# Kmatsuo57/cell-image-analysis

Hardware: AMD Instinct MI355X
Metric: cells/sec screened (CAE fwd + recon-MSE + SVM score), 64x64 (higher is better)
Workload: dtype f32 (results in the fp32 error class; the contractions run as split 16-bit products on the matrix pipe, fp32 accumulate: conv1..conv6 as 2 fp16 terms x 3 products with exact power-of-two scales from each cell's own data, the PCA GEMM as 3 bf16 terms x 6 products, conv7's 32 -> 16 channel contraction; 1 GPU; BASELINE.json configs[2]: screening inference, 1000000 synthetic 64x64 crops on one GPU, resident in HBM, CAE fwd + recon MSE/MAE + RobustScaler + PCA(100) + 2x OCSVM score on device; cells_per_gpu=1000000, global_cells=1000000, chunk_cells=65536, detector_train_cells=5000, weights=random init (Glorot, non-trivial BN), seed 42, parallelism=dp1

## Files before the change

cell-image-analysis_amd/cellscreen/_lib.py:

```python
from __future__ import annotations

import ctypes as C
import os
from typing import Optional

import numpy as np

CS_MAX_CONV = 16
CS_MEM_HOST, CS_MEM_DEVICE = 0, 1
_PKG = os.path.dirname(os.path.dirname(os.path.abspath(__file__)))
LIB_PATH = os.path.join(_PKG, "libcellscreen.so")


class CellScreenError(RuntimeError):
    def __init__(self, status: int, message: str):
        super().__init__(f"libcellscreen status {status}: {message}")
        self.status = status


class CSAugAffine(C.Structure):
    _fields_ = [("m", C.c_double * 4), ("off", C.c_double * 2), ("identity", C.c_int32), ("flip_h", C.c_int32),
                ("flip_v", C.c_int32), ("reserved", C.c_int32)]


# ... 178 lines not shown
                                   C.POINTER(CSBackgroundParams), _P, _I]),
    "cs_segment_background_last_timing": (_I, [_P, C.POINTER(C.c_double), C.POINTER(C.c_double)]),
    "cs_segment_local": (_I, [_P, _P, _I, C.c_int32, C.c_int32, C.c_int32, C.c_int32, C.c_int32, _I, C.POINTER(CSLocalParams), _P, _I]),
    "cs_segment_local_last_timing": (_I, [_P, C.POINTER(C.c_double), C.POINTER(C.c_double)]),
    "cs_segment_clean": (_I, [_P, _P, _I, C.c_int32, C.c_int32, C.c_int32, C.c_int32, C.c_int32, _I, C.POINTER(CSSegmentParams),
                              C.POINTER(CSCleanParams), _P, _I, _P]),
    "cs_segment_clean_last_timing": (_I, [_P, C.POINTER(C.c_double), C.POINTER(C.c_double), C.POINTER(C.c_double)]),
    "cs_segment_hysteresis": (_I, [_P, _P, _I, C.c_int32, C.c_int32, C.c_int32, C.c_int32, C.c_int32, _I, C.POINTER(CSSegmentParams),
                                   C.POINTER(CSLocalParams), C.POINTER(CSHysteresisParams), _P, _I, _P]),
    "cs_segment_hysteresis_last_timing": (_I, [_P, C.POINTER(C.c_double), C.POINTER(C.c_double)]),
    "cs_segment_noise": (_I, [_P, _P, _I, C.c_int32, C.c_int32, C.c_int32, C.c_int32, C.c_int32, _I, C.POINTER(CSNoiseParams), _P, _I, _P]),
    "cs_segment_noise_last_timing": (_I, [_P, C.POINTER(C.c_double), C.POINTER(C.c_double), C.POINTER(C.c_double)]),
    "cs_segment_smooth": (_I, [_P, _P, _I, C.c_int32, C.c_int32, C.c_int32, C.c_int32, C.c_int32, _I, C.POINTER(CSSmoothParams), _P, _I]),
    "cs_segment_smooth_last_timing": (_I, [_P, C.POINTER(C.c_double), C.POINTER(C.c_double)]),
    "cs_label_match": (_I, [_P, _P, _P, C.c_int32, C.c_int32, C.c_int32, _I, C.c_int32, C.c_int32, C.POINTER(CSMatchParams), _P, _P, _I, _P]),
    "cs_label_match_last_timing": (_I, [_P, C.POINTER(C.c_double), C.POINTER(C.c_double)]),
    "cs_label_match_last_table": (_I, [_P, C.POINTER(C.c_int32), C.POINTER(C.c_int32)]),
    "cs_label_expand": (_I, [_P, _P, C.c_int32, C.c_int32, C.c_int32, _I, C.POINTER(CSExpandParams), _P, _P, _I]),
    "cs_label_expand_last_timing": (_I, [_P, C.POINTER(C.c_double), C.POINTER(C.c_double)]),
    "cs_label_intensity": (_I, [_P, _P, _I, C.c_int32, _P, _P, C.c_int32, C.c_int32, C.c_int32, _I, C.c_int32, _P, _P, _I]),
    "cs_label_intensity_last_timing": (_I, [_P, C.POINTER(C.c_double), C.POINTER(C.c_double)]),
    "cs_label_quantiles": (_I, [_P, _P, _I, C.c_int32, _P, _P, C.c_int32, C.c_int32, C.c_int32, _I, C.c_int32, _P, _P, C.c_int32, _I,
                                _P, _P, _P, _I]),
    "cs_label_quantiles_last_timing": (_I, [_P, C.POINTER(C.c_double), C.POINTER(C.c_double), C.POINTER(C.c_double)]),
    "cs_label_texture": (_I, [_P, _P, _I, C.c_int32, _P, _P, C.c_int32, C.c_int32, C.c_int32, _I, C.c_int32, C.c_int32, C.c_int32, _P, _P,
                              _P, _P, _P, _P, _P, _I]),
    "cs_label_texture_last_timing": (_I, [_P, C.POINTER(C.c_double), C.POINTER(C.c_double)]),
    "cs_label_shape": (_I, [_P, _P, _P, C.c_int32, C.c_int32, C.c_int32, _I, C.c_int32, _I, _P, _P, _P, _P, _P, _I]),
    "cs_label_shape_last_timing": (_I, [_P, C.POINTER(C.c_double), C.POINTER(C.c_double)]),
    "cs_label_neighbors": (_I, [_P, _P, C.c_int32, C.c_int32, C.c_int32, _I, C.c_int32, C.POINTER(CSNeighborsParams), _P, _P, _P, _I,
                           C.POINTER(_L)]),
    "cs_label_neighbors_pairs": (_I, [_P, _P, _L, _I]),
    "cs_label_neighbors_last_timing": (_I, [_P, C.POINTER(C.c_double), C.POINTER(C.c_double)]),
    "cs_label_neighbors_last_table": (_I, [_P, C.POINTER(C.c_int32), C.POINTER(C.c_int32)]),
    "cs_fit_create": (_I, [_I, C.POINTER(_P)]),
    "cs_fit_free": (None, [_P]),
    "cs_fit_wait_stream": (_I, [_P, _P]),
    "cs_fit_scaler": (_I, [_P, _P, _L, C.c_int32, _I, _P, _P]),
    "cs_fit_pca_moments": (_I, [_P, _P, _L, C.c_int32, _I, _P, _P, _P, _P]),
    "cs_fit_pca_subspace": (_I, [_P, _P, _L, C.c_int32, _I, _P, _P, C.c_int32, C.c_uint64, _P, _P, _P, C.POINTER(C.c_double),
                                 C.POINTER(C.c_int32)]),
    "cs_fit_project": (_I, [_P, _P, _L, C.c_int32, _I, _P, _P, _P, _P, C.c_int32, _P]),
    "cs_fit_ocsvm": (_I, [_P, _P, _L, C.c_int32, C.c_double, C.c_double, C.c_double, _L, _P, C.POINTER(C.c_double),
                          C.POINTER(C.c_double), C.POINTER(_L), C.POINTER(C.c_int32)]),
    "cs_fit_last_ms": (_I, [_P, C.POINTER(C.c_double)]),
    "cs_synth_crops": (_I, [_P, C.c_uint64, _L, _L, C.c_int32, _P]),
    "cs_profile_enable": (_I, [_P, _I]),
    "cs_profile_reset": (_I, [_P]),
    "cs_profile_kernel_count": (_I, []),
    "cs_profile_kernel_name": (C.c_char_p, [_I]),
    "cs_profile_get": (_I, [_P, _I, C.POINTER(C.c_double), C.POINTER(_L), C.POINTER(_L), C.POINTER(C.c_double)]),
    "cs_profile_mfma_per_cell": (_I, [_P, _I, C.POINTER(C.c_double)]),
    "cs_profile_bf16_mfma_per_cell": (_I, [_P, _I, C.POINTER(C.c_double)]),
    "cs_train_param_count": (_I, [C.POINTER(_L), C.POINTER(_L)]),
    "cs_train_param_count_of": (_I, [_P, C.POINTER(_L), C.POINTER(_L)]),
    "cs_train_create": (_I, [C.POINTER(CSCaeWeights), C.POINTER(CSTrainCfg), _I, C.POINTER(_P)]),
    "cs_train_free": (None, [_P]),
    "cs_train_wait_stream": (_I, [_P, _P]),
    "cs_train_step": (_I, [_P, _P, _P, _L, _I, C.c_float, C.POINTER(C.c_float), C.POINTER(C.c_float)]),
    "cs_train_step_async": (_I, [_P, _P, _P, _L, _I, C.c_float]),
    "cs_train_inputs_consumed": (_I, [_P, _P]),
    "cs_train_draw_transforms": (_I, [C.POINTER(CSAugConfig), C.c_uint64, C.c_uint64, _L, C.c_int32, C.c_int32, _P]),
    "cs_train_fit_step": (_I, [_P, _P, _L, _P, _L, C.POINTER(CSAugConfig), C.c_uint64, C.c_uint64, C.c_float]),
    "cs_train_read_metrics": (_I, [_P, C.POINTER(C.c_double), C.POINTER(C.c_double), C.POINTER(_L), _I]),
    "cs_train_forward_backward": (_I, [_P, _P, _P, _L, _I, C.POINTER(C.c_float), C.POINTER(C.c_float)]),
    "cs_train_apply": (_I, [_P, C.c_float]),
    "cs_train_set_grad_buffer": (_I, [_P, _P]),
    "cs_train_set_sync_bn": (_I, [_P, _P, _P, _P, _L, _I, _I]),
    "cs_train_set_sync_bn_stream": (_I, [_P, _P, _P, _P, _L, _I, _I]),
    "cs_train_eval": (_I, [_P, _P, _P, _L, _I, C.POINTER(C.c_float), C.POINTER(C.c_float)]),
    "cs_train_augment": (_I, [_P, _P, _L, _P, _P, _I]),
    "cs_train_export": (_I, [_P, _P, _P, _P]),
    "cs_train_tensor": (_I, [_P, _I, _I, _L, _P]),
    "cs_train_import": (_I, [_P, _P, _P]),
}

_lib = None


def load_library(path: Optional[str] = None):
    global _lib
    if _lib is not None:
        return _lib
    path = path or LIB_PATH
    if not os.path.exists(path):
        raise FileNotFoundError(f"{path} not built; run `python cell-image-analysis_amd/build.py` "
                                "(or __graft_entry__.build()).  There is no CPU fallback.")
    try:
        import torch
    except Exception:
        pass
    lib = C.CDLL(path, mode=C.RTLD_GLOBAL)
    for name, (res, args) in SIGNATURES.items():
        fn = getattr(lib, name)
        fn.restype = res
        fn.argtypes = args
    if lib.cs_abi_version() != 2:
        raise RuntimeError("libcellscreen ABI version mismatch")
    _lib = lib
    return lib


def check(status: int):
    if status != 0:
        lib = load_library()
        msg = lib.cs_last_error().decode(errors="replace") or lib.cs_status_string(status).decode()
# ... 44 lines not shown
```

cell-image-analysis_amd/cellscreen/engine.py:

```python
from __future__ import annotations

import ctypes as C
from typing import Dict, Optional

import numpy as np

from . import _lib as L
from . import spec
from .spec import CAEWeights, DetectorParams


def _fill_cae(w: CAEWeights, keep: list) -> L.CSCaeWeights:
    s = L.CSCaeWeights()
    s.height, s.width = w.input_hw
    s.n_conv, s.n_enc = w.n_conv, w.n_enc
    s.bn_eps = w.bn_eps

    def put(field, l, arr):
        a = np.ascontiguousarray(arr, dtype=np.float32)
        keep.append(a)
        getattr(s, field)[l] = a.ctypes.data

    for l in range(w.n_conv):
        s.channels[l] = w.channels[l]
# ... 126 lines not shown

    def encode(self, crops, which: int = 1):
        buf, n, kind = self._crops(crops)
        f = self._alloc(kind, buf, (n, self.info.feature_dim), np.float32)
        L.check(self._lib.cs_encode(self._h, L._ptr(buf), n, kind, which, L._ptr(f), kind))
        return f

    def layer_output(self, crops, layer: int):
        buf, n, kind = self._crops(crops)
        rows = spec.layer_table((self.info.height, self.info.width), tuple(self.info.channels[:self.info.n_conv]), self.info.n_enc)
        oh, ow = rows[layer]["out_hw"]
        o = self._alloc(kind, buf, (n, oh, ow, rows[layer]["cout"]), np.float32)
        L.check(self._lib.cs_layer_output(self._h, L._ptr(buf), n, kind, layer, L._ptr(o), kind))
        return o

    def scaler_pca(self, features: np.ndarray) -> np.ndarray:
        f = np.ascontiguousarray(features, dtype=np.float32)
        o = np.empty((f.shape[0], self.info.n_components), dtype=np.float32)
        L.check(self._lib.cs_scaler_pca(self._h, f.ctypes.data, f.shape[0], L.CS_MEM_HOST, o.ctypes.data, L.CS_MEM_HOST))
        return o

    def svm_decision(self, pca: np.ndarray):
        p = np.ascontiguousarray(pca, dtype=np.float32)
        c = np.empty(p.shape[0], dtype=np.float64)
        m = np.empty(p.shape[0], dtype=np.float64)
        L.check(self._lib.cs_svm_decision(self._h, p.ctypes.data, p.shape[0], L.CS_MEM_HOST, c.ctypes.data, m.ctypes.data, L.CS_MEM_HOST))
        return c, m

    def synth_crops(self, seed: int, first_cell: int, out_tensor):
        n = out_tensor.shape[0]
        npix = int(np.prod(out_tensor.shape[1:]))
        L.order_after_torch(self._lib.cs_model_wait_stream, self._h, out_tensor)
        L.check(self._lib.cs_synth_crops(self._h, seed, first_cell, n, npix, out_tensor.data_ptr()))
        return out_tensor

    def profile_enable(self, on: bool = True):
        L.check(self._lib.cs_profile_enable(self._h, 1 if on else 0))

    def profile_reset(self):
        L.check(self._lib.cs_profile_reset(self._h))

    def profile(self) -> Dict[str, dict]:
        out = {}
        for k in range(self._lib.cs_profile_kernel_count()):
            ms, ln, cells, fl = C.c_double(), C.c_int64(), C.c_int64(), C.c_double()
            L.check(self._lib.cs_profile_get(self._h, k, C.byref(ms), C.byref(ln), C.byref(cells), C.byref(fl)))
            mf = C.c_double()
            L.check(self._lib.cs_profile_mfma_per_cell(self._h, k, C.byref(mf)))
            bf = C.c_double()
            L.check(self._lib.cs_profile_bf16_mfma_per_cell(self._h, k, C.byref(bf)))
            out[self._lib.cs_profile_kernel_name(k).decode()] = dict(ms=ms.value, launches=ln.value, cells=cells.value, flops=fl.value,
                                                                      mfma_per_cell=mf.value, bf16_mfma_per_cell=bf.value)
        return out
```

cell-image-analysis_amd/csrc/api.hip:

```cpp
#include "api_internal.hpp"
#include "tensor_archive.hpp"

using namespace cs;

static thread_local std::string g_err;

namespace cs {
int fail(int code, const char* fmt, ...)
{
    char buf[1024];
    va_list ap;
    va_start(ap, fmt);
    vsnprintf(buf, sizeof buf, fmt, ap);
    va_end(ap);
    g_err = buf;
    return code;
}
const char* last_error_cstr() { return g_err.c_str(); }
}

static const char* kKernelNames[K_COUNT] = {"conv1_relu_bn_pool", "conv2_relu_bn_pool", "conv3_relu_bn_pool",
                                            "conv4_relu_bn",      "conv5_up_relu_bn",   "conv6_up_relu_bn",
                                            "conv7_up_sigmoid_err", "scaler_pca",       "ocsvm_decision",
                                            "finalize",           "synth_crops",        "conv6_conv7_fused_err",
// ... 1143 lines not shown
    if ((rc = ensure_workspace(m, ch, false))) return rc;
    double* outs[2] = {cons_dec, mod_dec};
    for (int64_t off = 0; off < n; off += ch) {
        const int64_t nc = (n - off) < ch ? (n - off) : ch;
        const float* p;
        if ((rc = stage_in(m, pca, in_kind, off, nc, (size_t)m->C, m->pca, &p))) return rc;
        for (int d = 0; d < 2; ++d) {
            if (!outs[d]) continue;
            LAUNCH(K_SVM, nc,
                   launch_ocsvm(p, m->C, m->svm[d].svT.as<double>(), m->svm[d].svn.as<double>(), m->svm[d].coef.as<double>(),
                                m->svm[d].nsv_pad, m->svm[d].gamma, m->svm[d].rho, m->dec[d].as<double>(), nc, m->stream, m->det_ws.p));
            HIPCHK(hipMemcpyAsync(outs[d] + off, m->dec[d].p, (size_t)nc * sizeof(double),
                                  out_kind == CS_MEM_DEVICE ? hipMemcpyDeviceToDevice : hipMemcpyDeviceToHost, m->stream));
        }
        HIPCHK(hipStreamSynchronize(m->stream));
    }
    return guard.done(end_call(m));
}

int cs_synth_crops(cs_model* m, uint64_t seed, int64_t first_cell, int64_t n, int32_t npix, float* out_device)
{
    int rc = begin_call(m);
    if (rc) return rc;
    if (n < 0 || npix <= 0) return fail(CS_ERR_INVALID, "n/npix invalid");
    if (n == 0) return CS_OK;
    if (!out_device) return fail(CS_ERR_INVALID, "out_device is NULL");
    LAUNCH(K_SYNTH, n, launch_synth(seed, first_cell, n, npix, out_device, m->stream));
    return end_call(m);
}

int cs_profile_enable(cs_model* m, int on)
{
    if (!m) return fail(CS_ERR_INVALID, "model handle is NULL");
    m->prof = on != 0;
    return CS_OK;
}

int cs_profile_reset(cs_model* m)
{
    if (!m) return fail(CS_ERR_INVALID, "model handle is NULL");
    for (int k = 0; k < K_COUNT; ++k) { m->prof_ms[k] = 0; m->prof_launches[k] = 0; m->prof_cells[k] = 0; }
    return CS_OK;
}

int cs_model_wait_stream(cs_model* m, void* hip_stream)
{
    if (!m) return fail(CS_ERR_INVALID, "model handle is NULL");
    HIPCHK(hipSetDevice(m->device));
    return wait_on_stream(m->stream, hip_stream);
}

int cs_profile_kernel_count(void) { return K_COUNT; }

const char* cs_profile_kernel_name(int k) { return (k >= 0 && k < K_COUNT) ? kKernelNames[k] : ""; }

int cs_profile_get(cs_model* m, int k, double* total_ms, int64_t* launches, int64_t* cells, double* flops)
{
    if (!m || k < 0 || k >= K_COUNT) return fail(CS_ERR_INVALID, "bad kernel id");
    if (total_ms) *total_ms = m->prof_ms[k];
    if (launches) *launches = m->prof_launches[k];
    if (cells) *cells = m->prof_cells[k];
    if (flops) {
        double per_cell = 0.0;
        if (k <= K_CONV7_ERR) per_cell = 2.0 * kLayerMacs[k];
        else if (k == K_CONV67_FUSED) per_cell = 2.0 * (kLayerMacs[5] + kLayerMacs[6]);
        else if (k == K_CONV12_FUSED) per_cell = 2.0 * (kLayerMacs[0] + kLayerMacs[1]);
        else if (k == K_SCALER_PCA) per_cell = 2.0 * (double)m->F * m->C;
        else if (k == K_SVM) per_cell = 0.0;
        *flops = per_cell * (double)m->prof_cells[k];
    }
    return CS_OK;
}

int cs_profile_mfma_per_cell(cs_model* m, int k, double* mfma)
{
    if (!m || !mfma || k < 0 || k >= K_COUNT) return fail(CS_ERR_INVALID, "bad kernel id");
    double v = 0.0;
    if (k == K_SCALER_PCA) {
        *mfma = m->has_det && !m->split16 ? (double)m->fpad * m->cpad / 1024.0 : 0.0;
        return CS_OK;
    }
    if (m->arch.ref) {
        const bool h2 = m->split16;
        switch (k) {
            case K_CONV1: v = 1536; break;
            case K_CONV2: v = 8192; break;
            case K_CONV3: v = h2 ? 0 : 2048; break;
            case K_CONV4: v = h2 ? 0 : 576; break;
            case K_CONV5: v = h2 ? 0 : 1152; break;
            case K_CONV6: v = 4608; break;
            case K_CONV67_FUSED: v = h2 ? 512 : 4608 + 512; break;
            case K_CONV12_FUSED: v = h2 ? 0 : 4608 + 1536 + 48; break;
            default: v = 0.0;
        }
    } else if (k <= K_CONV6 || k == K_CONV7_ERR) {
        const int l = k == K_CONV7_ERR ? m->arch.n_conv - 1 : k - K_CONV1;
        if (l < m->arch.n_conv && !(m->split16 && m->gae.x3[l])) {
            const int cout_pad = (m->arch.ch[l] + 15) / 16 * 16;
            v = (double)m->arch.gh[l] * m->arch.gw[l] / 16.0 * (cout_pad / 16) * (9.0 * m->arch.cin(l) / 4.0);
        }
    }
    *mfma = v;
    return CS_OK;
}

int cs_profile_bf16_mfma_per_cell(cs_model* m, int k, double* mfma)
// ... 29 lines not shown
```

cell-image-analysis_amd/csrc/common.hpp:

```cpp
#pragma once
#include <hip/hip_runtime.h>
#include <stdint.h>
#include <stdio.h>

#include "../../include/cellscreen.h"

namespace cs {

typedef float f32x4 __attribute__((ext_vector_type(4)));

struct LayerGeom {
    int H, W, cin, cout;
    bool pool;
    bool ups;
    bool last;
};

enum KernelId {
    K_CONV1 = 0, K_CONV2, K_CONV3, K_CONV4, K_CONV5, K_CONV6, K_CONV7_ERR,
    K_SCALER_PCA, K_SVM, K_FINALIZE, K_SYNTH, K_CONV67_FUSED, K_CONV12_FUSED, K_COUNT
};

hipError_t launch_conv_mfma(int layer, const float* in, const float* wfrag, const float* ep,
                            float* out, int64_t n_cells, hipStream_t stream, bool folded = false);
size_t pack_conv_fragments_folded(int cin, int cout, const float* hwio, float* dst);
hipError_t launch_conv_wino_cs(int layer, const float* in, const float* ufrag, const float* ep, float* out, int64_t n_cells,
                               hipStream_t stream);
size_t pack_wino_cs_fragments(int layer, const float* hwio, float* dst);
hipError_t launch_conv3_wino_h2(const float* in, const uint16_t* uplanes, float inv_sw, const float* ep, float* out, int64_t n_cells,
                                hipStream_t stream);
size_t pack_wino3_h2(const float* hwio, uint16_t* dst, float* inv_sw);
hipError_t launch_conv12_fused(const float* x, const float* w1frag, const float* ep1, const float* ufrag, const float* ep2, float* p2,
                               int64_t n_cells, hipStream_t stream, const unsigned int* ufrag_h2 = nullptr,
                               float p1a = 0.0f, float p1b = 0.0f, float inv_sw = 1.0f, const unsigned int* w1h2 = nullptr, float inv_sw1 = 1.0f);
size_t pack_conv12_conv1_h2(const float* hwio, const float* bn_scale, unsigned int* dst, float* inv_sw1);
size_t pack_conv12_fragments_h2(const float* hwio, const float* bn_scale, unsigned int* dst, float* inv_sw);
void pack_conv12_p1_bound(const float* hwio1, const float* ep1, float* a1, float* b1);
size_t pack_conv12_fragments(const float* hwio, const float* bn_scale, float* dst);
size_t pack_conv12_conv1_fragments(const float* hwio, const float* bn_scale, float* dst);
hipError_t launch_conv4_h2(const float* in, const uint16_t* wfrag, float inv_sw, const float* ep, float* out, int64_t n_cells, hipStream_t stream);
size_t pack_conv4_f16x2(const float* hwio, uint16_t* dst, float* inv_sw);
hipError_t launch_conv5_h2(const float* in, const uint16_t* wfrag, float inv_sw, const float* ep, float* out, int64_t n_cells, hipStream_t stream);
hipError_t launch_conv45_h2(const float* in, const uint16_t* w4, float inv_sw4, const float* ep4, const uint16_t* w5, float inv_sw5,
                            const float* ep5, float* out, int64_t n_cells, hipStream_t stream);
size_t pack_conv5_f16x2(const float* weff, uint16_t* dst, float* inv_sw);
hipError_t launch_conv_wino_up(int layer, const float* in, const float* ufrag, const float* ep, float* out, int64_t n_cells,
                               hipStream_t stream);
size_t pack_wino_up_fragments(int layer, const float* hwio, float* dst);
size_t pack_conv_fragments(int cin, int cout, const float* hwio, float* dst);

hipError_t launch_conv67_fused(const float* a5, const float* ufrag, const float* ep, const float* x, const float* weff_dev,
                               const float* b7_dev, float* errpart, int64_t n_cells, hipStream_t stream);
int conv67_fused_nparts();
hipError_t launch_conv67_h2(const float* a5, const uint16_t* wplanes, float inv_sw, const float* ep, const float* x, const float* weff_dev,
                            const float* b7_dev, float* errpart, int64_t n_cells, hipStream_t stream);
size_t pack_conv6_f16x2(const float* weff, uint16_t* dst, float* inv_sw);

hipError_t launch_conv7_err(const float* a6, const float* x, const float* weff_dev, const float* b7_dev,
                            float* errpart, float* recon, int64_t n_cells, hipStream_t stream);
hipError_t launch_conv7_err_train(const float* a6, const float* x, const float* weff_dev, const float* b7_dev, float* errpart,
                                  float* recon, float* dz, float* dzsum_part, int64_t n_cells, hipStream_t stream);
void conv7_effective_weights(const float* w7_hwio, float* weff);

constexpr int TRAIN_MAX_PARTS = 256;
constexpr int BN_MAX_PARTS = 1024;
struct ReduceDesc { long dst; long len; const float* src; int nparts; long stride; };
hipError_t launch_conv_train_fwd(int layer, const float* in, const float* wfrag, const float* bias,
                                 float* relu_out, int64_t n_cells, hipStream_t stream, float* stats_part = nullptr,
                                 int* stats_parts = nullptr);
hipError_t launch_conv_dgrad(int layer, const float* dz, const float* wfrag_t, float* dx, int64_t n_cells,
                             hipStream_t stream);
hipError_t launch_bn_stats(const float* r, long P, int C, float* part, int* G, hipStream_t s);
hipError_t launch_bn_stats_final(const float* part, int G, int C, float eps, float momentum, float* mov_mean,
                                 float* mov_var, float* stats, hipStream_t s);
hipError_t launch_bn_stats_merge(const float* part, int G, int C, float* out , hipStream_t s);
hipError_t launch_bn_apply(const float* r, int C, const float* gamma, const float* beta, const float* stats, float* a,
                           long N, int H, int W, int pool, hipStream_t s);
hipError_t launch_loss_dz(const float* out, const float* y, long total, float* dz, float* dzsum_part, int* G, hipStream_t s,
                          const float* errpart = nullptr, long nparts = 0, float* out2 = nullptr);
hipError_t launch_loss_scalar(const float* errpart, long nparts, long nelem, float* out2, hipStream_t s);
hipError_t launch_bn_bwd_reduce(const float* da, const float* r, const float* stats, const float* gamma, const float* beta,
                                long N, int H, int W, int C, int pool, float* part, int* G, hipStream_t s);
hipError_t launch_bn_bwd_final(const float* part, int G, int C, double nred, float* sums, float* dgamma, float* dbeta,
                               hipStream_t s);
hipError_t launch_bn_bwd_dz(const float* da, const float* r, const float* stats, const float* gamma, const float* beta,
                            const float* sums, long N, int H, int W, int C, int pool, float* dz, float* dzsum_part,
                            int* Gz, hipStream_t s);
hipError_t launch_wgrad(int layer, const float* xin, const float* dz, float* part, int64_t n_cells, int* nparts,
                        hipStream_t s);
hipError_t launch_reduce_all(const ReduceDesc* descs_dev, int ndesc, long total_len, float* flat_grad, hipStream_t s,
                             const float* errpart = nullptr, long nparts = 0, long nelem = 0, float* out2 = nullptr);
hipError_t launch_adam(float* p, const float* g, float* m, float* v, long n, float alpha, float b1, float b2, float eps, hipStream_t s,
                       const float* batch_scal, double* macc);
enum { GEN_EPI_BN = 0, GEN_EPI_BN_POOL = 1, GEN_EPI_SIGMOID = 2, GEN_EPI_RELU = 3, GEN_EPI_PLAIN = 4 };
int conv_generic_supported(int H, int W, int cin, int cout, char* why, size_t why_len);
hipError_t launch_conv_generic(const float* in, const float* w_hwio, const float* ep, float* out, int64_t n, int H, int W, int cin,
                               int cout, int ups, int epi, hipStream_t stream, const float* w_folded = nullptr);
// ... 58 lines not shown
```

cell-image-analysis_amd/csrc/conv45_h2.hip:

```cpp
#include "kernel_setup.hpp"
#include "split16.hpp"

#include <cstring>

namespace cs {

namespace {

constexpr int G = 8;
constexpr int CH = 32;
constexpr int WP = G + 2;
constexpr int PXB = 64;
constexpr int ROWB = WP * PXB + 32;
constexpr int PLANE = WP * ROWB;
constexpr int WG_PER_CU = 2;

constexpr int C5_OUT = 64;

constexpr int H2_OFF_MAX = 2 * PLANE;
constexpr int H2_LDS_BYTES = 2 * PLANE + 16;

__device__ __forceinline__ void h2_split_store(char* dst, const f32x4& x, float S)
{
    f16x4 hi;
// ... 139 lines not shown
    __syncthreads();
    float S, invS;
    f16x2_scale(mxw[0], S, invS);
    const int woff = ((tid >> 6) + 1) * ROWB + (((tid >> 3) & 7) + 1) * PXB + (tid & 7) * 8;
    const int abase = ((li >> 3) + pa) * ROWB + ((li & 7) + pb) * PXB + kq * 16;

    for (int it = 0; cell < n_cells; cell += gridDim.x, ++it) {
        const float unscale = invS * inv_sw;
        h2_split_store(smem + woff, stg, S);
        __syncthreads();
        if (tid == 0) mxw[it & 1] = 0;
        const long ncell = cell + gridDim.x;
        if (ncell < n_cells) stg = *(const f32x4*)(in + (size_t)ncell * (G * G * CH) + tid * 4);

        float* obase = out + (((size_t)cell * (2 * G) + pa) * (2 * G) + pb) * C5_OUT + (2 * sp) * 16 + li;
#pragma unroll
        for (int t = 0; t < 4; ++t) {
            f32x4 ah[2] = {{0.0f, 0.0f, 0.0f, 0.0f}, {0.0f, 0.0f, 0.0f, 0.0f}};
            f32x4 al[2] = {{0.0f, 0.0f, 0.0f, 0.0f}, {0.0f, 0.0f, 0.0f, 0.0f}};
#pragma unroll
            for (int tap = 0; tap < 4; ++tap) {
                const char* a = smem + abase + t * (2 * ROWB) + (tap >> 1) * ROWB + (tap & 1) * PXB;
                const f16x8 a1 = *(const f16x8*)a;
                const f16x8 a2 = *(const f16x8*)(a + PLANE);
#pragma unroll
                for (int k = 0; k < 2; ++k) {
                    al[k] = __builtin_amdgcn_mfma_f32_16x16x32_f16(a1, B[tap][k][1], al[k], 0, 0, 0);
                    ah[k] = __builtin_amdgcn_mfma_f32_16x16x32_f16(a1, B[tap][k][0], ah[k], 0, 0, 0);
                    al[k] = __builtin_amdgcn_mfma_f32_16x16x32_f16(a2, B[tap][k][0], al[k], 0, 0, 0);
                }
            }
#pragma unroll
            for (int r = 0; r < 4; ++r) {
                const int i = 4 * kq + r, ys = 2 * t + (i >> 3), xs = i & 7;
                float* o = obase + ((size_t)(2 * ys) * (2 * G) + 2 * xs) * C5_OUT;
#pragma unroll
                for (int k = 0; k < 2; ++k) {
                    const float v = fmaxf(fmaf(ah[k][r] + al[k][r], unscale, bias[k]), 0.0f);
                    o[16 * k] = fmaf(v, bns[k], bnt[k]);
                }
            }
        }
        if (ncell < n_cells) {
            unsigned int mx = 0;
            f16x2_absmax4(stg, mx);
            mx = f16x2_rowmax(mx);
            if (li == 0) atomicMax(&mxw[(it + 1) & 1], mx);
        }
        __syncthreads();
        f16x2_scale(mxw[(it + 1) & 1], S, invS);
    }
}

constexpr int F45_OFF_A = 2 * PLANE;
constexpr int F45_OFF_W4 = 4 * PLANE;
constexpr int F45_W4_BYTES = 2 * 9 * 2 * 64 * 16;
constexpr int F45_OFF_MAX = F45_OFF_W4 + F45_W4_BYTES;
constexpr int F45_LDS_BYTES = F45_OFF_MAX + 16;
static_assert(2 * F45_LDS_BYTES <= 160 * 1024, "two workgroups per CU");

__global__ __launch_bounds__(512, 2) void conv45_h2_kernel(const float* __restrict__ in , const f16x8* __restrict__ w4frag,
                                                           const float* __restrict__ ep4, float inv_sw4, const f16x8* __restrict__ w5frag,
                                                           const float* __restrict__ ep5, float inv_sw5, float* __restrict__ out ,
                                                           long n_cells)
{
    extern __shared__ __attribute__((aligned(16))) char smem[];
    unsigned int* const mxw = (unsigned int*)(smem + F45_OFF_MAX);
    const int tid = threadIdx.x;
    const int lane = tid & 63;
    const int wave = __builtin_amdgcn_readfirstlane(tid >> 6);
    const int li = lane & 15, kq = lane >> 4;
    const int ph = wave >> 1, pa = ph >> 1, pb = ph & 1;
    const int sp = wave & 1;
    const int slice4 = wave & 1, tile4 = wave >> 1;

    f16x8 B[4][2][2];
#pragma unroll
    for (int t = 0; t < 4; ++t)
#pragma unroll
        for (int k = 0; k < 2; ++k)
#pragma unroll
            for (int p = 0; p < 2; ++p) B[t][k][p] = w5frag[(((wave * 4 + t) * 2 + k) * 2 + p) * 64 + lane];
    float bias[2], bns[2], bnt[2];
#pragma unroll
    for (int k = 0; k < 2; ++k) {
        const int co = (2 * sp + k) * 16 + li;
        bias[k] = ep5[co]; bns[k] = ep5[C5_OUT + co]; bnt[k] = ep5[2 * C5_OUT + co];
    }
    const int co4 = slice4 * 16 + li;
    const float bias4 = ep4[co4], bns4 = ep4[CH + co4], bnt4 = ep4[2 * CH + co4];

    for (int i = tid; i < F45_LDS_BYTES / 16; i += 512) *(f32x4*)(smem + i * 16) = f32x4{0.0f, 0.0f, 0.0f, 0.0f};
    __syncthreads();
    for (int i = tid; i < F45_W4_BYTES / 16; i += 512) *(f16x8*)(smem + F45_OFF_W4 + i * 16) = w4frag[i];

    long cell = blockIdx.x;
    if (cell >= n_cells) return;
    f32x4 stg = *(const f32x4*)(in + (size_t)cell * (G * G * CH) + tid * 4);
    {
        unsigned int mx = 0;
        f16x2_absmax4(stg, mx);
        mx = f16x2_rowmax(mx);
        if (li == 0) atomicMax(&mxw[0], mx);
    }
    __syncthreads();
    float S3, invS3;
    f16x2_scale(mxw[0], S3, invS3);
    const int woff = ((tid >> 6) + 1) * ROWB + (((tid >> 3) & 7) + 1) * PXB + (tid & 7) * 8;
    const int abase4 = (2 * tile4 + (li >> 3)) * ROWB + (li & 7) * PXB + kq * 16;
    const char* const w4l = smem + F45_OFF_W4 + (size_t)slice4 * 9 * 2 * 64 * 16 + lane * 16;
    const int abase5 = F45_OFF_A + ((li >> 3) + pa) * ROWB + ((li & 7) + pb) * PXB + kq * 16;

    for (int it = 0; cell < n_cells; cell += gridDim.x, ++it) {
        h2_split_store(smem + woff, stg, S3);
        __syncthreads();
        if (tid == 0) mxw[it & 1] = 0;
        const long ncell = cell + gridDim.x;
        if (ncell < n_cells) stg = *(const f32x4*)(in + (size_t)ncell * (G * G * CH) + tid * 4);

        f32x4 a4v;
        {
            f32x4 hi = {0.0f, 0.0f, 0.0f, 0.0f}, lo = {0.0f, 0.0f, 0.0f, 0.0f};
#pragma unroll
            for (int tap = 0; tap < 9; ++tap) {
                const char* a = smem + abase4 + (tap / 3) * ROWB + (tap % 3) * PXB;
                const f16x8 a1 = *(const f16x8*)a;
                const f16x8 a2 = *(const f16x8*)(a + PLANE);
                const f16x8 bh = *(const f16x8*)(w4l + (tap * 2 + 0) * 1024), bl = *(const f16x8*)(w4l + (tap * 2 + 1) * 1024);
                lo = __builtin_amdgcn_mfma_f32_16x16x32_f16(a1, bl, lo, 0, 0, 0);
                hi = __builtin_amdgcn_mfma_f32_16x16x32_f16(a1, bh, hi, 0, 0, 0);
                lo = __builtin_amdgcn_mfma_f32_16x16x32_f16(a2, bh, lo, 0, 0, 0);
            }
            const float us4 = invS3 * inv_sw4;
            float am = 0.0f;
#pragma unroll
            for (int r = 0; r < 4; ++r) {
                const float v = fmaxf(fmaf(hi[r] + lo[r], us4, bias4), 0.0f);
                a4v[r] = fmaf(v, bns4, bnt4);
                am = fmaxf(am, fabsf(a4v[r]));
            }
            const unsigned int m = f16x2_rowmax(__builtin_bit_cast(unsigned int, am));
            if (li == 0) atomicMax(&mxw[2 + (it & 1)], m);
        }
        __syncthreads();
        float S4, invS4;
        f16x2_scale(mxw[2 + (it & 1)], S4, invS4);
        {
#pragma unroll
            for (int r = 0; r < 4; ++r) {
                const int p = 16 * tile4 + 4 * kq + r;
                char* d = smem + F45_OFF_A + ((p >> 3) + 1) * ROWB + ((p & 7) + 1) * PXB + co4 * 2;
                const float v = a4v[r] * S4;
                const _Float16 h = (_Float16)v;
                *(_Float16*)d = h;
                *(_Float16*)(d + PLANE) = (_Float16)(v - (float)h);
            }
        }
        __syncthreads();
        if (tid == 0) mxw[2 + (it & 1)] = 0;

        const float unscale = invS4 * inv_sw5;
        float* obase = out + (((size_t)cell * (2 * G) + pa) * (2 * G) + pb) * C5_OUT + (2 * sp) * 16 + li;
#pragma unroll
        for (int t = 0; t < 4; ++t) {
            f32x4 ah[2] = {{0.0f, 0.0f, 0.0f, 0.0f}, {0.0f, 0.0f, 0.0f, 0.0f}};
            f32x4 al[2] = {{0.0f, 0.0f, 0.0f, 0.0f}, {0.0f, 0.0f, 0.0f, 0.0f}};
#pragma unroll
            for (int tap = 0; tap < 4; ++tap) {
                const char* a = smem + abase5 + t * (2 * ROWB) + (tap >> 1) * ROWB + (tap & 1) * PXB;
                const f16x8 a1 = *(const f16x8*)a;
                const f16x8 a2 = *(const f16x8*)(a + PLANE);
#pragma unroll
                for (int k = 0; k < 2; ++k) {
                    al[k] = __builtin_amdgcn_mfma_f32_16x16x32_f16(a1, B[tap][k][1], al[k], 0, 0, 0);
                    ah[k] = __builtin_amdgcn_mfma_f32_16x16x32_f16(a1, B[tap][k][0], ah[k], 0, 0, 0);
                    al[k] = __builtin_amdgcn_mfma_f32_16x16x32_f16(a2, B[tap][k][0], al[k], 0, 0, 0);
                }
            }
#pragma unroll
            for (int r = 0; r < 4; ++r) {
                const int i = 4 * kq + r, ys = 2 * t + (i >> 3), xs = i & 7;
                float* o = obase + ((size_t)(2 * ys) * (2 * G) + 2 * xs) * C5_OUT;
#pragma unroll
                for (int k = 0; k < 2; ++k) {
                    const float v = fmaxf(fmaf(ah[k][r] + al[k][r], unscale, bias[k]), 0.0f);
                    o[16 * k] = fmaf(v, bns[k], bnt[k]);
                }
            }
        }
        if (ncell < n_cells) {
            unsigned int mx = 0;
            f16x2_absmax4(stg, mx);
            mx = f16x2_rowmax(mx);
            if (li == 0) atomicMax(&mxw[(it + 1) & 1], mx);
        }
        __syncthreads();
        f16x2_scale(mxw[(it + 1) & 1], S3, invS3);
    }
}

}

size_t pack_conv4_f16x2(const float* hwio, uint16_t* dst, float* inv_sw)
{
    const size_t n = (size_t)2 * 9 * 2 * 64 * 8;
    if (!dst) return n;
    const float S = f16x2_weight_scale(hwio, (size_t)9 * CH * CH);
    if (inv_sw) *inv_sw = 1.0f / S;
    for (int s = 0; s < 2; ++s)
        for (int t = 0; t < 9; ++t)
            for (int l = 0; l < 64; ++l)
                for (int j = 0; j < 8; ++j) {
                    const int li = l & 15, kq = l >> 4;
                    uint16_t pl[2];
                    f16x2_split(hwio[((size_t)t * CH + 8 * kq + j) * CH + 16 * s + li], S, pl[0], pl[1]);
                    for (int p = 0; p < 2; ++p) dst[((((size_t)s * 9 + t) * 2 + p) * 64 + l) * 8 + j] = pl[p];
                }
    return n;
}

hipError_t launch_conv4_h2(const float* in, const uint16_t* wfrag, float inv_sw, const float* ep, float* out, int64_t n_cells, hipStream_t stream)
{
    if (n_cells <= 0) return hipSuccess;
    KernelSetup ks;
    if (hipError_t e = kernel_setup<conv4_h2_kernel>(256, H2_LDS_BYTES, ks); e != hipSuccess) return e;
    const long grid = n_cells < ks.resident ? n_cells : ks.resident;
    hipLaunchKernelGGL(conv4_h2_kernel, dim3((unsigned)grid), dim3(256), H2_LDS_BYTES, stream, in, (const f16x8*)wfrag, ep, out,
                       (long)n_cells, inv_sw);
    return hipGetLastError();
}

size_t pack_conv5_f16x2(const float* weff, uint16_t* dst, float* inv_sw)
{
    const size_t n = (size_t)8 * 4 * 2 * 2 * 64 * 8;
    if (!dst) return n;
    const float S = f16x2_weight_scale(weff, (size_t)16 * CH * C5_OUT);
    if (inv_sw) *inv_sw = 1.0f / S;
    for (int w = 0; w < 8; ++w)
        for (int t = 0; t < 4; ++t)
            for (int k = 0; k < 2; ++k)
                for (int l = 0; l < 64; ++l)
                    for (int j = 0; j < 8; ++j) {
                        const int ph = w >> 1, sp = w & 1, li = l & 15, kq = l >> 4;
                        uint16_t pl[2];
                        f16x2_split(weff[((size_t)(ph * 4 + t) * CH + 8 * kq + j) * C5_OUT + (2 * sp + k) * 16 + li], S, pl[0], pl[1]);
                        for (int p = 0; p < 2; ++p) dst[((((((size_t)w * 4 + t) * 2 + k) * 2 + p) * 64) + l) * 8 + j] = pl[p];
                    }
    return n;
}

hipError_t launch_conv5_h2(const float* in, const uint16_t* wfrag, float inv_sw, const float* ep, float* out, int64_t n_cells, hipStream_t stream)
{
    if (n_cells <= 0) return hipSuccess;
    KernelSetup ks;
    if (hipError_t e = kernel_setup<conv5_h2_kernel>(512, H2_LDS_BYTES, ks); e != hipSuccess) return e;
    const long grid = n_cells < ks.resident ? n_cells : ks.resident;
    hipLaunchKernelGGL(conv5_h2_kernel, dim3((unsigned)grid), dim3(512), H2_LDS_BYTES, stream, in, (const f16x8*)wfrag, ep, out,
                       (long)n_cells, inv_sw);
    return hipGetLastError();
}

hipError_t launch_conv45_h2(const float* in, const uint16_t* w4, float inv_sw4, const float* ep4, const uint16_t* w5, float inv_sw5,
                            const float* ep5, float* out, int64_t n_cells, hipStream_t stream)
{
    if (n_cells <= 0) return hipSuccess;
    KernelSetup ks;
    if (hipError_t e = kernel_setup<conv45_h2_kernel>(512, F45_LDS_BYTES, ks); e != hipSuccess) return e;
    const long grid = n_cells < ks.resident ? n_cells : ks.resident;
    hipLaunchKernelGGL(conv45_h2_kernel, dim3((unsigned)grid), dim3(512), F45_LDS_BYTES, stream, in, (const f16x8*)w4, ep4, inv_sw4,
                       (const f16x8*)w5, ep5, inv_sw5, out, (long)n_cells);
    return hipGetLastError();
}

}
```

include/cellscreen.h:

```cpp
#ifndef CELLSCREEN_H
#define CELLSCREEN_H

#include <stdint.h>

#ifdef __cplusplus
extern "C" {
#endif

#define CS_ABI_VERSION 2
#define CS_MAX_CONV 16

typedef enum cs_status {
    CS_OK = 0,
    CS_ERR_INVALID = -1,
    CS_ERR_IO = -2,
    CS_ERR_FORMAT = -3,
    CS_ERR_NO_DEVICE = -4,
    CS_ERR_HIP = -5,
    CS_ERR_UNSUPPORTED = -6,
    CS_ERR_NOMEM = -7,
    CS_ERR_NO_DETECTOR = -8
} cs_status;

typedef enum cs_mem_kind { CS_MEM_HOST = 0, CS_MEM_DEVICE = 1 } cs_mem_kind;
// ... 280 lines not shown
                       int32_t batch, int32_t height, int32_t width, int in_kind, int32_t max_label,
                       const int32_t *q_num, const int32_t *q_den, int32_t n_q, int want_mad,
                       int32_t *count, int32_t *order, int32_t *mad , int out_kind);
int cs_label_quantiles_last_timing(const cs_preproc *p, double *count_ms, double *scatter_ms, double *select_ms);

int cs_label_texture(cs_preproc *p, const void *image, int pixel_type, int32_t channels,
                     const int32_t *labels, const int32_t *exclude ,
                     int32_t batch, int32_t height, int32_t width, int in_kind, int32_t max_label,
                     int32_t levels, int32_t distance, const int32_t *range_lo, const int32_t *range_hi,
                     int32_t *count, int32_t *marg, int64_t *sumsq, double *clogc, int32_t *glcm , int out_kind);
int cs_label_texture_last_timing(const cs_preproc *p, double *boxes_ms, double *matrices_ms);

int cs_label_shape(cs_preproc *p, const int32_t *labels, const int32_t *exclude ,
                   int32_t batch, int32_t height, int32_t width, int in_kind, int32_t max_label, int want_hull,
                   int64_t *moments, int32_t *box, int32_t *quads, int32_t *perim, int64_t *hull , int out_kind);
int cs_label_shape_last_timing(const cs_preproc *p, double *moments_ms, double *outline_ms);

typedef struct cs_neighbors_params {
    int32_t max_d2;
    int32_t table_log2;
    int32_t reserved;
} cs_neighbors_params;
int cs_label_neighbors(cs_preproc *p, const int32_t *labels, int32_t batch, int32_t height, int32_t width, int in_kind,
                       int32_t max_label, const cs_neighbors_params *params, int64_t *geom, int32_t *objects, int64_t *offsets,
                       int out_kind, int64_t *n_pairs);
int cs_label_neighbors_pairs(cs_preproc *p, int32_t *pairs, int64_t capacity, int pairs_kind);
int cs_label_neighbors_last_timing(const cs_preproc *p, double *scan_ms, double *rows_ms);
int cs_label_neighbors_last_table(const cs_preproc *p, int32_t *table_log2, int32_t *grows);

typedef struct cs_fit cs_fit;
int cs_fit_create(int device_id, cs_fit **out);
void cs_fit_free(cs_fit *f);
int cs_fit_wait_stream(cs_fit *f, void *hip_stream);
int cs_fit_scaler(cs_fit *f, const float *features, int64_t n, int32_t n_features, int kind, float *center, double *scale);
int cs_fit_pca_moments(cs_fit *f, const float *features, int64_t n, int32_t n_features, int kind, const float *center,
                       const double *scale, float *mean, double *scatter);
int cs_fit_pca_subspace(cs_fit *f, const float *features, int64_t n, int32_t n_features, int kind, const float *center,
                        const double *scale, int32_t n_components, uint64_t seed, float *mean, double *components,
                        double *explained_variance, double *total_variance, int32_t *n_iter);
int cs_fit_project(cs_fit *f, const float *features, int64_t n, int32_t n_features, int kind, const float *center,
                   const double *scale, const float *components, const float *mean_proj, int32_t n_components, float *out);
int cs_fit_ocsvm(cs_fit *f, const double *x, int64_t n, int32_t n_components, double gamma, double nu, double eps,
                 int64_t max_iter, double *alpha, double *rho, double *obj, int64_t *n_iter, int32_t *status);
int cs_fit_last_ms(const cs_fit *f, double *device_ms);

int cs_profile_enable(cs_model *m, int on);
int cs_profile_reset(cs_model *m);
int cs_profile_kernel_count(void);
const char *cs_profile_kernel_name(int kernel_id);
int cs_profile_get(cs_model *m, int kernel_id, double *total_ms, int64_t *launches,
                   int64_t *cells, double *flops);
int cs_profile_mfma_per_cell(cs_model *m, int kernel_id, double *mfma);
int cs_profile_bf16_mfma_per_cell(cs_model *m, int kernel_id, double *mfma);

typedef struct cs_trainer cs_trainer;

typedef struct cs_train_cfg {
    float beta1, beta2, adam_eps;
    float bn_momentum, bn_eps;
} cs_train_cfg;

int cs_train_param_count(int64_t *n_trainable, int64_t *n_moving);
int cs_train_param_count_of(const cs_trainer *t, int64_t *n_trainable, int64_t *n_moving);
int cs_train_create(const cs_cae_weights *init, const cs_train_cfg *cfg, int device_id, cs_trainer **out);
void cs_train_free(cs_trainer *t);
int cs_train_wait_stream(cs_trainer *t, void *hip_stream);
int cs_train_step(cs_trainer *t, const float *x, const float *y, int64_t batch, int kind, float lr,
                  float *loss, float *mae);
int cs_train_step_async(cs_trainer *t, const float *x, const float *y, int64_t batch, int kind, float lr);
int cs_train_inputs_consumed(cs_trainer *t, void *hip_stream);
int cs_train_read_metrics(cs_trainer *t, double *loss_mean, double *mae_mean, int64_t *steps, int reset);
int cs_train_forward_backward(cs_trainer *t, const float *x, const float *y, int64_t batch, int kind,
                              float *loss, float *mae);
int cs_train_apply(cs_trainer *t, float lr);
typedef int (*cs_allgather_fn)(void *ctx, int64_t floats_per_rank);
int cs_train_set_sync_bn(cs_trainer *t, cs_allgather_fn fn, void *ctx, float *device_buf, int64_t capacity_floats, int rank, int world);
typedef int (*cs_allgather_stream_fn)(void *ctx, int64_t floats_per_rank, void *hip_stream);
int cs_train_set_sync_bn_stream(cs_trainer *t, cs_allgather_stream_fn fn, void *ctx, float *device_buf, int64_t capacity_floats,
                                int rank, int world);
int cs_train_set_grad_buffer(cs_trainer *t, float *device_buffer);
int cs_train_eval(cs_trainer *t, const float *x, const float *y, int64_t n, int kind, float *loss, float *mae);
typedef struct cs_aug_affine {
    double m[4];
    double off[2];
    int32_t identity, flip_h, flip_v, reserved;
} cs_aug_affine;
int cs_train_augment(cs_trainer *t, const float *x, int64_t n, const cs_aug_affine *tf, float *out, int kind);

typedef struct cs_aug_config {
    double rotation_range;
    double width_shift_range, height_shift_range;
    double zoom_lo, zoom_hi;
    int32_t horizontal_flip, vertical_flip;
    double center;
} cs_aug_config;
int cs_train_draw_transforms(const cs_aug_config *aug, uint64_t seed, uint64_t step, int64_t n, int32_t height, int32_t width,
                             cs_aug_affine *out);
int cs_train_fit_step(cs_trainer *t, const float *train_device, int64_t n_train, const int32_t *idx, int64_t batch,
                      const cs_aug_config *aug, uint64_t seed, uint64_t step, float lr);

int cs_train_export(cs_trainer *t, float *params_host, float *moving_host, float *grads_host);
int cs_train_tensor(cs_trainer *t, int which, int layer, int64_t batch, float *host);
int cs_train_import(cs_trainer *t, const float *params_host, const float *moving_host);

#ifdef __cplusplus
}
// ... 3 lines not shown
```

Before: 5.590 million cells/s.

## Process two cells per pass in fused conv4+conv5 kernel to share weight loads

The fused conv4+conv5 kernel now holds two cells per workgroup pass in LDS, sharing the conv4 weight fragment loads across both cells and halving the barriers per cell. LDS per workgroup roughly doubles, so occupancy drops from two workgroups per CU to one. A query for the resident grid size is exposed through the C API and Python. The trade is fewer barriers and weight reloads against lower occupancy and higher register pressure.

Result: no change. 5.564 million cells/s (median of 2 runs) (-0.5%).

```diff
diff --git a/cell-image-analysis_amd/cellscreen/_lib.py b/cell-image-analysis_amd/cellscreen/_lib.py
--- a/cell-image-analysis_amd/cellscreen/_lib.py
+++ b/cell-image-analysis_amd/cellscreen/_lib.py
@@ -254,6 +254,7 @@
     "cs_profile_get": (_I, [_P, _I, C.POINTER(C.c_double), C.POINTER(_L), C.POINTER(_L), C.POINTER(C.c_double)]),
     "cs_profile_mfma_per_cell": (_I, [_P, _I, C.POINTER(C.c_double)]),
     "cs_profile_bf16_mfma_per_cell": (_I, [_P, _I, C.POINTER(C.c_double)]),
+    "cs_profile_conv45_grid": (_I, [_P, C.POINTER(C.c_int32)]),
     "cs_train_param_count": (_I, [C.POINTER(_L), C.POINTER(_L)]),
     "cs_train_param_count_of": (_I, [_P, C.POINTER(_L), C.POINTER(_L)]),
     "cs_train_create": (_I, [C.POINTER(CSCaeWeights), C.POINTER(CSTrainCfg), _I, C.POINTER(_P)]),
diff --git a/cell-image-analysis_amd/cellscreen/engine.py b/cell-image-analysis_amd/cellscreen/engine.py
--- a/cell-image-analysis_amd/cellscreen/engine.py
+++ b/cell-image-analysis_amd/cellscreen/engine.py
@@ -202,3 +202,8 @@
             out[self._lib.cs_profile_kernel_name(k).decode()] = dict(ms=ms.value, launches=ln.value, cells=cells.value, flops=fl.value,
                                                                       mfma_per_cell=mf.value, bf16_mfma_per_cell=bf.value)
         return out
+
+    def conv45_grid(self) -> int:
+        g = C.c_int32()
+        L.check(self._lib.cs_profile_conv45_grid(self._h, C.byref(g)))
+        return g.value
diff --git a/cell-image-analysis_amd/csrc/api.hip b/cell-image-analysis_amd/csrc/api.hip
--- a/cell-image-analysis_amd/csrc/api.hip
+++ b/cell-image-analysis_amd/csrc/api.hip
@@ -1219,6 +1219,17 @@
 
 int cs_profile_kernel_count(void) { return K_COUNT; }
 
+int cs_profile_conv45_grid(cs_model* m, int32_t* workgroups)
+{
+    if (!m || !workgroups) return fail(CS_ERR_INVALID, "model handle or result pointer is NULL");
+    if (!m->arch.ref || !m->split16) return fail(CS_ERR_UNSUPPORTED, "the fused conv4 + conv5 kernel belongs to the reference graph in split16");
+    HIPCHK(hipSetDevice(m->device));
+    int g = 0;
+    HIPCHK(conv45_h2_max_grid(&g));
+    *workgroups = g;
+    return CS_OK;
+}
+
 const char* cs_profile_kernel_name(int k) { return (k >= 0 && k < K_COUNT) ? kKernelNames[k] : ""; }
 
 int cs_profile_get(cs_model* m, int k, double* total_ms, int64_t* launches, int64_t* cells, double* flops)
diff --git a/cell-image-analysis_amd/csrc/common.hpp b/cell-image-analysis_amd/csrc/common.hpp
--- a/cell-image-analysis_amd/csrc/common.hpp
+++ b/cell-image-analysis_amd/csrc/common.hpp
@@ -43,6 +43,7 @@
 hipError_t launch_conv5_h2(const float* in, const uint16_t* wfrag, float inv_sw, const float* ep, float* out, int64_t n_cells, hipStream_t stream);
 hipError_t launch_conv45_h2(const float* in, const uint16_t* w4, float inv_sw4, const float* ep4, const uint16_t* w5, float inv_sw5,
                             const float* ep5, float* out, int64_t n_cells, hipStream_t stream);
+hipError_t conv45_h2_max_grid(int* workgroups);
 size_t pack_conv5_f16x2(const float* weff, uint16_t* dst, float* inv_sw);
 hipError_t launch_conv_wino_up(int layer, const float* in, const float* ufrag, const float* ep, float* out, int64_t n_cells,
                                hipStream_t stream);
diff --git a/cell-image-analysis_amd/csrc/conv45_h2.hip b/cell-image-analysis_amd/csrc/conv45_h2.hip
--- a/cell-image-analysis_amd/csrc/conv45_h2.hip
+++ b/cell-image-analysis_amd/csrc/conv45_h2.hip
@@ -215,12 +215,15 @@
     }
 }
 
-constexpr int F45_OFF_A = 2 * PLANE;
-constexpr int F45_OFF_W4 = 4 * PLANE;
+constexpr int F45_IMG = 2 * PLANE;
+constexpr int F45_OFF_A = 2 * F45_IMG;
+constexpr int F45_OFF_W4 = 4 * F45_IMG;
 constexpr int F45_W4_BYTES = 2 * 9 * 2 * 64 * 16;
 constexpr int F45_OFF_MAX = F45_OFF_W4 + F45_W4_BYTES;
-constexpr int F45_LDS_BYTES = F45_OFF_MAX + 16;
-static_assert(2 * F45_LDS_BYTES <= 160 * 1024, "two workgroups per CU");
+constexpr int F45_LDS_BYTES = F45_OFF_MAX + 32;
+static_assert(F45_LDS_BYTES <= 160 * 1024, "one workgroup per CU: 4 images of 13,440 B + 36,864 B of conv4 weights + 32 B of maxima");
+
+template <int N> struct PassCells { static constexpr int value = N; };
 
 __global__ __launch_bounds__(512, 2) void conv45_h2_kernel(const float* __restrict__ in , const f16x8* __restrict__ w4frag,
                                                            const float* __restrict__ ep4, float inv_sw4, const f16x8* __restrict__ w5frag,
@@ -257,108 +260,150 @@
     __syncthreads();
     for (int i = tid; i < F45_W4_BYTES / 16; i += 512) *(f16x8*)(smem + F45_OFF_W4 + i * 16) = w4frag[i];
 
-    long cell = blockIdx.x;
-    if (cell >= n_cells) return;
-    f32x4 stg = *(const f32x4*)(in + (size_t)cell * (G * G * CH) + tid * 4);
-    {
-        unsigned int mx = 0;
-        f16x2_absmax4(stg, mx);
-        mx = f16x2_rowmax(mx);
-        if (li == 0) atomicMax(&mxw[0], mx);
-    }
-    __syncthreads();
-    float S3, invS3;
-    f16x2_scale(mxw[0], S3, invS3);
+    const long stride = gridDim.x;
+    long cell[2] = {(long)blockIdx.x, (long)blockIdx.x + stride};
+    if (cell[0] >= n_cells) return;
+    f32x4 stg[2] = {{0.0f, 0.0f, 0.0f, 0.0f}, {0.0f, 0.0f, 0.0f, 0.0f}};
+#pragma unroll
+    for (int c = 0; c < 2; ++c) {
+        if (cell[c] < n_cells) {
+            stg[c] = *(const f32x4*)(in + (size_t)cell[c] * (G * G * CH) + tid * 4);
+            unsigned int mx = 0;
+            f16x2_absmax4(stg[c], mx);
+            mx = f16x2_rowmax(mx);
+            if (li == 0) atomicMax(&mxw[c], mx);
+        }
+    }
+    __syncthreads();
+    float S3[2], invS3[2];
+#pragma unroll
+    for (int c = 0; c < 2; ++c) f16x2_scale(mxw[c], S3[c], invS3[c]);
     const int woff = ((tid >> 6) + 1) * ROWB + (((tid >> 3) & 7) + 1) * PXB + (tid & 7) * 8;
     const int abase4 = (2 * tile4 + (li >> 3)) * ROWB + (li & 7) * PXB + kq * 16;
     const char* const w4l = smem + F45_OFF_W4 + (size_t)slice4 * 9 * 2 * 64 * 16 + lane * 16;
     const int abase5 = F45_OFF_A + ((li >> 3) + pa) * ROWB + ((li & 7) + pb) * PXB + kq * 16;
 
-    for (int it = 0; cell < n_cells; cell += gridDim.x, ++it) {
-        h2_split_store(smem + woff, stg, S3);
-        __syncthreads();
-        if (tid == 0) mxw[it & 1] = 0;
-        const long ncell = cell + gridDim.x;
-        if (ncell < n_cells) stg = *(const f32x4*)(in + (size_t)ncell * (G * G * CH) + tid * 4);
-
-        f32x4 a4v;
+    auto pass = [&](auto nc, const int par) __attribute__((always_inline)) {
+        constexpr int NC = decltype(nc)::value;
+        unsigned int* const mxp = mxw + 2 * par;
+        unsigned int* const mxa = mxw + 4 + 2 * par;
+        unsigned int* const mxn = mxw + 2 * (par ^ 1);
+#pragma unroll
+        for (int c = 0; c < NC; ++c) h2_split_store(smem + c * F45_IMG + woff, stg[c], S3[c]);
+        __syncthreads();
+        if (tid < NC) mxp[tid] = 0;
+        long ncell[2] = {cell[0] + 2 * stride, cell[1] + 2 * stride};
+        if constexpr (NC == 2) {
+#pragma unroll
+            for (int c = 0; c < 2; ++c)
+                if (ncell[c] < n_cells) stg[c] = *(const f32x4*)(in + (size_t)ncell[c] * (G * G * CH) + tid * 4);
+        }
+
+        f32x4 a4v[NC];
         {
-            f32x4 hi = {0.0f, 0.0f, 0.0f, 0.0f}, lo = {0.0f, 0.0f, 0.0f, 0.0f};
+            f32x4 hi[NC], lo[NC];
+#pragma unroll
+            for (int c = 0; c < NC; ++c) hi[c] = lo[c] = f32x4{0.0f, 0.0f, 0.0f, 0.0f};
 #pragma unroll
             for (int tap = 0; tap < 9; ++tap) {
-                const char* a = smem + abase4 + (tap / 3) * ROWB + (tap % 3) * PXB;
-                const f16x8 a1 = *(const f16x8*)a;
-                const f16x8 a2 = *(const f16x8*)(a + PLANE);
                 const f16x8 bh = *(const f16x8*)(w4l + (tap * 2 + 0) * 1024), bl = *(const f16x8*)(w4l + (tap * 2 + 1) * 1024);
-                lo = __builtin_amdgcn_mfma_f32_16x16x32_f16(a1, bl, lo, 0, 0, 0);
-                hi = __builtin_amdgcn_mfma_f32_16x16x32_f16(a1, bh, hi, 0, 0, 0);
-                lo = __builtin_amdgcn_mfma_f32_16x16x32_f16(a2, bh, lo, 0, 0, 0);
-            }
-            const float us4 = invS3 * inv_sw4;
-            float am = 0.0f;
-#pragma unroll
-            for (int r = 0; r < 4; ++r) {
-                const float v = fmaxf(fmaf(hi[r] + lo[r], us4, bias4), 0.0f);
-                a4v[r] = fmaf(v, bns4, bnt4);
-                am = fmaxf(am, fabsf(a4v[r]));
-            }
-            const unsigned int m = f16x2_rowmax(__builtin_bit_cast(unsigned int, am));
-            if (li == 0) atomicMax(&mxw[2 + (it & 1)], m);
-        }
-        __syncthreads();
-        float S4, invS4;
-        f16x2_scale(mxw[2 + (it & 1)], S4, invS4);
-        {
+#pragma unroll
+                for (int c = 0; c < NC; ++c) {
+                    const char* a = smem + c * F45_IMG + abase4 + (tap / 3) * ROWB + (tap % 3) * PXB;
+                    const f16x8 a1 = *(const f16x8*)a;
+                    const f16x8 a2 = *(const f16x8*)(a + PLANE);
+                    lo[c] = __builtin_amdgcn_mfma_f32_16x16x32_f16(a1, bl, lo[c], 0, 0, 0);
+                    hi[c] = __builtin_amdgcn_mfma_f32_16x16x32_f16(a1, bh, hi[c], 0, 0, 0);
+                    lo[c] = __builtin_amdgcn_mfma_f32_16x16x32_f16(a2, bh, lo[c], 0, 0, 0);
+                }
+            }
+#pragma unroll
+            for (int c = 0; c < NC; ++c) {
+                const float us4 = invS3[c] * inv_sw4;
+                float am = 0.0f;
+#pragma unroll
+                for (int r = 0; r < 4; ++r) {
+                    const float v = fmaxf(fmaf(hi[c][r] + lo[c][r], us4, bias4), 0.0f);
+                    a4v[c][r] = fmaf(v, bns4, bnt4);
+                    am = fmaxf(am, fabsf(a4v[c][r]));
+                }
+                const unsigned int m = f16x2_rowmax(__builtin_bit_cast(unsigned int, am));
+                if (li == 0) atomicMax(&mxa[c], m);
+            }
+        }
+        __syncthreads();
+        float invS4[NC];
+#pragma unroll
+        for (int c = 0; c < NC; ++c) {
+            float S4;
+            f16x2_scale(mxa[c], S4, invS4[c]);
 #pragma unroll
             for (int r = 0; r < 4; ++r) {
                 const int p = 16 * tile4 + 4 * kq + r;
-                char* d = smem + F45_OFF_A + ((p >> 3) + 1) * ROWB + ((p & 7) + 1) * PXB + co4 * 2;
-                const float v = a4v[r] * S4;
+                char* d = smem + F45_OFF_A + c * F45_IMG + ((p >> 3) + 1) * ROWB + ((p & 7) + 1) * PXB + co4 * 2;
+                const float v = a4v[c][r] * S4;
                 const _Float16 h = (_Float16)v;
                 *(_Float16*)d = h;
                 *(_Float16*)(d + PLANE) = (_Float16)(v - (float)h);
             }
         }
         __syncthreads();
-        if (tid == 0) mxw[2 + (it & 1)] = 0;
-
-        const float unscale = invS4 * inv_sw5;
-        float* obase = out + (((size_t)cell * (2 * G) + pa) * (2 * G) + pb) * C5_OUT + (2 * sp) * 16 + li;
-#pragma unroll
-        for (int t = 0; t < 4; ++t) {
-            f32x4 ah[2] = {{0.0f, 0.0f, 0.0f, 0.0f}, {0.0f, 0.0f, 0.0f, 0.0f}};
-            f32x4 al[2] = {{0.0f, 0.0f, 0.0f, 0.0f}, {0.0f, 0.0f, 0.0f, 0.0f}};
-#pragma unroll
-            for (int tap = 0; tap < 4; ++tap) {
-                const char* a = smem + abase5 + t * (2 * ROWB) + (tap >> 1) * ROWB + (tap & 1) * PXB;
-                const f16x8 a1 = *(const f16x8*)a;
-                const f16x8 a2 = *(const f16x8*)(a + PLANE);
-#pragma unroll
-                for (int k = 0; k < 2; ++k) {
-                    al[k] = __builtin_amdgcn_mfma_f32_16x16x32_f16(a1, B[tap][k][1], al[k], 0, 0, 0);
-                    ah[k] = __builtin_amdgcn_mfma_f32_16x16x32_f16(a1, B[tap][k][0], ah[k], 0, 0, 0);
-                    al[k] = __builtin_amdgcn_mfma_f32_16x16x32_f16(a2, B[tap][k][0], al[k], 0, 0, 0);
-                }
-            }
-#pragma unroll
-            for (int r = 0; r < 4; ++r) {
-                const int i = 4 * kq + r, ys = 2 * t + (i >> 3), xs = i & 7;
-                float* o = obase + ((size_t)(2 * ys) * (2 * G) + 2 * xs) * C5_OUT;
-#pragma unroll
-                for (int k = 0; k < 2; ++k) {
-                    const float v = fmaxf(fmaf(ah[k][r] + al[k][r], unscale, bias[k]), 0.0f);
-                    o[16 * k] = fmaf(v, bns[k], bnt[k]);
-                }
-            }
-        }
-        if (ncell < n_cells) {
-            unsigned int mx = 0;
-            f16x2_absmax4(stg, mx);
-            mx = f16x2_rowmax(mx);
-            if (li == 0) atomicMax(&mxw[(it + 1) & 1], mx);
-        }
-        __syncthreads();
-        f16x2_scale(mxw[(it + 1) & 1], S3, invS3);
+        if (tid < NC) mxa[tid] = 0;
+
+#pragma unroll
+        for (int c = 0; c < NC; ++c) {
+            const float unscale = invS4[c] * inv_sw5;
+            float* obase = out + (((size_t)cell[c] * (2 * G) + pa) * (2 * G) + pb) * C5_OUT + (2 * sp) * 16 + li;
+#pragma unroll
+            for (int t = 0; t < 4; ++t) {
+                f32x4 ah[2] = {{0.0f, 0.0f, 0.0f, 0.0f}, {0.0f, 0.0f, 0.0f, 0.0f}};
+                f32x4 al[2] = {{0.0f, 0.0f, 0.0f, 0.0f}, {0.0f, 0.0f, 0.0f, 0.0f}};
+#pragma unroll
+                for (int tap = 0; tap < 4; ++tap) {
+                    const char* a = smem + c * F45_IMG + abase5 + t * (2 * ROWB) + (tap >> 1) * ROWB + (tap & 1) * PXB;
+                    const f16x8 a1 = *(const f16x8*)a;
+                    const f16x8 a2 = *(const f16x8*)(a + PLANE);
+#pragma unroll
+                    for (int k = 0; k < 2; ++k) {
+                        al[k] = __builtin_amdgcn_mfma_f32_16x16x32_f16(a1, B[tap][k][1], al[k], 0, 0, 0);
+                        ah[k] = __builtin_amdgcn_mfma_f32_16x16x32_f16(a1, B[tap][k][0], ah[k], 0, 0, 0);
+                        al[k] = __builtin_amdgcn_mfma_f32_16x16x32_f16(a2, B[tap][k][0], al[k], 0, 0, 0);
+                    }
+                }
+#pragma unroll
+                for (int r = 0; r < 4; ++r) {
+                    const int i = 4 * kq + r, ys = 2 * t + (i >> 3), xs = i & 7;
+                    float* o = obase + ((size_t)(2 * ys) * (2 * G) + 2 * xs) * C5_OUT;
+#pragma unroll
+                    for (int k = 0; k < 2; ++k) {
+                        const float v = fmaxf(fmaf(ah[k][r] + al[k][r], unscale, bias[k]), 0.0f);
+                        o[16 * k] = fmaf(v, bns[k], bnt[k]);
+                    }
+                }
+            }
+        }
+        if constexpr (NC == 2) {
+#pragma unroll
+            for (int c = 0; c < 2; ++c) {
+                if (ncell[c] < n_cells) {
+                    unsigned int mx = 0;
+                    f16x2_absmax4(stg[c], mx);
+                    mx = f16x2_rowmax(mx);
+                    if (li == 0) atomicMax(&mxn[c], mx);
+                }
+            }
+        }
+        __syncthreads();
+#pragma unroll
+        for (int c = 0; c < 2; ++c) {
+            f16x2_scale(mxn[c], S3[c], invS3[c]);
+            cell[c] = ncell[c];
+        }
+    };
+
+    for (int it = 0; cell[0] < n_cells; ++it) {
+        if (cell[1] < n_cells) pass(PassCells<2>{}, it & 1);
+        else pass(PassCells<1>{}, it & 1);
     }
 }
 
@@ -435,4 +480,12 @@
     return hipGetLastError();
 }
 
-}
+hipError_t conv45_h2_max_grid(int* workgroups)
+{
+    KernelSetup ks;
+    if (hipError_t e = kernel_setup<conv45_h2_kernel>(512, F45_LDS_BYTES, ks); e != hipSuccess) return e;
+    *workgroups = ks.resident;
+    return hipSuccess;
+}
+
+}
diff --git a/include/cellscreen.h b/include/cellscreen.h
--- a/include/cellscreen.h
+++ b/include/cellscreen.h
@@ -356,6 +356,7 @@
                    int64_t *cells, double *flops);
 int cs_profile_mfma_per_cell(cs_model *m, int kernel_id, double *mfma);
 int cs_profile_bf16_mfma_per_cell(cs_model *m, int kernel_id, double *mfma);
+int cs_profile_conv45_grid(cs_model *m, int32_t *workgroups);
 
 typedef struct cs_trainer cs_trainer;
 
```
